# youmi-zym/TemporalStereo

Hardware: AMD Instinct MI355X
Metric: stereo pairs/sec, FlyingThings3D 540x960 D=192 (aggregation hot path) (higher is better)
Workload: dtype f32

## Files before the change

### include/ts_hip.h

```cpp
#ifndef TS_HIP_H
#define TS_HIP_H

#include <stddef.h>
#include <stdint.h>

#ifdef __cplusplus
extern "C" {
#endif

#define TS_OK 0
#define TS_ERR_NULL (-1)
#define TS_ERR_SHAPE (-2)
#define TS_ERR_UNSUPPORTED (-3)
#define TS_ERR_ALIGN (-4)

int ts_version(void);
const char* ts_last_error_string(void);

size_t ts_block_cost_workspace_bytes(int B, int C, int H, int W, int D, int scales);

int ts_block_cost_int_fwd(const float* left, const float* right, float* out, void* workspace,
                          int B, int C, int H, int W, int D, int scales, void* stream);

int ts_block_cost_sampled_fwd(const float* left, const float* right, const float* disp, float* out,
// ... 377 lines not shown
                          long long dx_bstride, long long dx_cstride, void* stream);
int ts_conv3d_hw_bwd_weight(const float* x, const float* dy, float* dw, int B, int Cin, int Cout, int D, int H, int W,
                            int stride, int dilation, long long x_bstride, long long x_cstride, long long dy_bstride,
                            long long dy_cstride, void* workspace, size_t workspace_bytes, void* stream);
int ts_conv3d_d_bwd_data(const float* dy, const float* w_b, float* dx, int B, int Cin, int Cout, int Din, int H, int W,
                         int k, int stride, int dilation, int padding, int transposed, long long dy_bstride,
                         long long dy_cstride, long long dx_bstride, long long dx_cstride, void* stream);
int ts_conv3d_d_bwd_weight(const float* x, const float* dy, float* dw, int B, int Cin, int Cout, int Din, int H, int W,
                           int k, int stride, int dilation, int padding, long long x_bstride, long long x_cstride,
                           long long dy_bstride, long long dy_cstride, void* workspace, size_t workspace_bytes,
                           void* stream);
int ts_resize3d_add_act_fwd(const float* a, const float* add, float* out, int B, int C, int Da, int Ha, int Wa,
                            int D, int H, int W, int act, long long a_bstride, long long a_cstride,
                            long long add_bstride, long long add_cstride, long long out_bstride,
                            long long out_cstride, void* stream);
int ts_pool3d5_avgmax_fwd(const float* x, float* out_avg, float* out_max, int B, int C, int D, int H, int W,
                          long long x_bstride, long long x_cstride, long long avg_bstride, long long avg_cstride,
                          long long max_bstride, long long max_cstride, void* stream);
int ts_merge_candidates_fwd(const float* volume, const float* sample, const float* mem_sample, const float* mem_cost,
                            const float* past_w, const float* past_scale, const float* past_shift,
                            float* out_sample, float* out_volume, int B, int C, int D0, int K, int H, int W,
                            long long vol_bstride, long long vol_cstride, long long out_bstride,
                            long long out_cstride, void* stream);
int ts_convex_upsample_fwd(const float* mask, const float* disp, float* out, int B, int H, int W, int factor,
                           float disp_scale, void* stream);
int ts_convex_upsample_candidates_fwd(const float* mask, const float* disp, float* out, float* low, float* high,
                                      float* candidates, int B, int H, int W, int factor, float disp_scale, float range,
                                      int channel_offset, int channels_total, void* stream);
int ts_unet_upsample_fwd(const float* mask, const float* disp, float* out, int B, int h, int w, int Ho, int Wo,
                         void* stream);
int ts_convex_upsample_bwd(const float* mask, const float* disp, const float* grad_out, float* grad_mask, float* grad_disp,
                           int B, int H, int W, int factor, float disp_scale, void* stream);
int ts_unet_upsample_bwd(const float* mask, const float* disp, const float* grad_out, float* grad_mask, float* grad_disp,
                         void* workspace, int B, int h, int w, int Ho, int Wo, void* stream);
int ts_deconv2d_k4s2_fwd(const float* x, const float* w_t, const float* scale, const float* shift, float* y,
                         int B, int Cin, int Cout, int H, int W, int act, long long out_bstride, void* stream);
int ts_resize_bilinear_fwd(const float* x, float* out, int B, int C, int h, int w, int Ho, int Wo, float value_scale,
                           long long out_bstride, void* stream);
int ts_resize_bilinear_pair_fwd(const float* x0, const float* x1, float* out0, float* out1, int B, int C, int h, int w,
                                int Ho, int Wo, float value_scale0, float value_scale1, void* stream);
int ts_range_candidates_fwd(const float* disp, float* low, float* high, float* candidates, int B, int H, int W,
                            float range, int channel_offset, int channels_total, void* stream);

int ts_resize3d_add_act_bwd(const float* a, const float* add, const float* grad_out, float* grad_a, float* grad_add,
                            int B, int C, int Da, int Ha, int Wa, int D, int H, int W, int act, void* stream);
int ts_pool3d5_avgmax_bwd(const float* x, const float* grad_avg, const float* grad_max, float* grad_x,
// ... 43 lines not shown
```

### temporalstereo_amd/_lib.py

```python
import ctypes
import os
import threading

_HERE = os.path.dirname(os.path.abspath(__file__))
LIB_PATH = os.path.join(_HERE, "libts_hip.so")

_lock = threading.Lock()
_lib = None

c_f32p = ctypes.c_void_p
c_ptr = ctypes.c_void_p
c_int = ctypes.c_int
c_size = ctypes.c_size_t
c_float = ctypes.c_float

SIGNATURES = {
    "ts_version": (c_int, []),
    "ts_last_error_string": (ctypes.c_char_p, []),
    "ts_block_cost_workspace_bytes": (c_size, [c_int] * 6),
    "ts_block_cost_int_fwd": (c_int, [c_f32p, c_f32p, c_f32p, c_ptr] + [c_int] * 6 + [c_ptr]),
    "ts_block_cost_sampled_fwd": (c_int, [c_f32p, c_f32p, c_f32p, c_f32p, c_ptr] + [c_int] * 6 + [c_ptr]),
    "ts_block_cost_sampled_warped_fwd": (c_int, [c_f32p, c_f32p, c_f32p, c_f32p, c_ptr] + [c_int] * 6 + [c_ptr]),
    "ts_block_cost_sampled_corr_fwd": (c_int, [c_f32p, c_f32p, c_f32p, c_f32p, c_ptr] + [c_int] * 6 + [c_ptr]),
    "ts_block_cost_corr_split_supported": (c_int, [c_int] * 2),
# ... 103 lines not shown
    "ts_conv3d_hw_x6_weight_bytes": (ctypes.c_size_t, [c_int] * 2),
    "ts_conv3d_hw_x6_weight_split": (c_int, [c_f32p, c_ptr, c_int, c_int, c_ptr]),
    "ts_conv3d_hw_x6_weight_split_from": (c_int, [c_f32p, c_ptr, c_int, c_int] + [ctypes.c_longlong] * 3 + [c_int, c_ptr]),
    "ts_conv3d_hw_x6_workspace_bytes": (c_size, [c_int] * 6),
    "ts_conv3d_hw_x6s_supported": (c_int, [c_int] * 5),
    "ts_conv3d_hw_x6s_weight_bytes": (c_size, [c_int] * 3),
    "ts_conv3d_hw_x6s_weight_split": (c_int, [c_f32p, c_ptr, c_int, c_int, c_int, c_int, c_ptr]),
    "ts_conv3d_hw_x6s_fwd": (c_int, [c_f32p, c_ptr, c_f32p, c_f32p, c_f32p] + [c_int] * 8 + [c_float] + [ctypes.c_longlong] * 4 + [c_ptr]),
    "ts_deconv2d_k4s2_unet_upsample_fwd": (c_int, [c_f32p, c_ptr, c_f32p, c_f32p, c_f32p, c_f32p] + [c_int] * 5 + [ctypes.c_longlong] * 2 + [c_ptr]),
    "ts_conv3d_hw_x6_fwd": (c_int, [c_f32p, c_ptr, c_f32p, c_f32p, c_f32p] + [c_int] * 8 + [c_float] + [ctypes.c_longlong] * 4 +
                            [c_f32p, ctypes.c_longlong, c_ptr, c_size, c_ptr]),
    "ts_conv3d_hw_fwd": (c_int, [c_f32p] * 5 + [c_int] * 10 + [c_float] + [ctypes.c_longlong] * 4 +
                         [c_f32p, ctypes.c_longlong, c_ptr, c_size, c_ptr]),
    "ts_conv3d_hw_workspace_bytes": (c_size, [c_int] * 8),
    "ts_conv3d_hw_bwd_data": (c_int, [c_f32p] * 3 + [c_int] * 9 + [ctypes.c_longlong] * 4 + [c_ptr]),
    "ts_conv3d_bwd_weight_workspace_bytes": (ctypes.c_size_t, [c_int] * 3),
    "ts_conv3d_hw_bwd_weight": (c_int, [c_f32p] * 3 + [c_int] * 8 + [ctypes.c_longlong] * 4 + [c_ptr, ctypes.c_size_t, c_ptr]),
    "ts_conv3d_d_bwd_data": (c_int, [c_f32p] * 3 + [c_int] * 11 + [ctypes.c_longlong] * 4 + [c_ptr]),
    "ts_conv3d_d_bwd_weight": (c_int, [c_f32p] * 3 + [c_int] * 10 + [ctypes.c_longlong] * 4 + [c_ptr, ctypes.c_size_t, c_ptr]),
    "ts_conv3d_d_fwd": (c_int, [c_f32p] * 5 + [c_int] * 12 + [c_float] + [ctypes.c_longlong] * 4 + [c_ptr]),
    "ts_resize3d_add_act_fwd": (c_int, [c_f32p] * 3 + [c_int] * 9 + [ctypes.c_longlong] * 6 + [c_ptr]),
    "ts_pool3d5_avgmax_fwd": (c_int, [c_f32p] * 3 + [c_int] * 5 + [ctypes.c_longlong] * 6 + [c_ptr]),
    "ts_merge_candidates_fwd": (c_int, [c_f32p] * 9 + [c_int] * 6 + [ctypes.c_longlong] * 4 + [c_ptr]),
    "ts_convex_upsample_fwd": (c_int, [c_f32p] * 3 + [c_int] * 4 + [c_float, c_ptr]),
    "ts_convex_upsample_candidates_fwd": (c_int, [c_f32p] * 6 + [c_int] * 4 + [c_float, c_float, c_int, c_int, c_ptr]),
    "ts_unet_upsample_fwd": (c_int, [c_f32p] * 3 + [c_int] * 5 + [c_ptr]),
    "ts_convex_upsample_bwd": (c_int, [c_f32p] * 5 + [c_int] * 4 + [c_float, c_ptr]),
    "ts_unet_upsample_bwd": (c_int, [c_f32p] * 5 + [c_ptr] + [c_int] * 5 + [c_ptr]),
    "ts_deconv2d_k4s2_fwd": (c_int, [c_f32p] * 5 + [c_int] * 6 + [ctypes.c_longlong, c_ptr]),
    "ts_resize_bilinear_fwd": (c_int, [c_f32p] * 2 + [c_int] * 6 + [c_float, ctypes.c_longlong, c_ptr]),
    "ts_resize_bilinear_pair_fwd": (c_int, [c_f32p] * 4 + [c_int] * 6 + [c_float, c_float, c_ptr]),
    "ts_range_candidates_fwd": (c_int, [c_f32p] * 4 + [c_int] * 3 + [c_float, c_int, c_int, c_ptr]),
    "ts_project_to_3d_fwd": (c_int, [c_f32p] * 7 + [c_int] * 6 + [c_float, c_ptr]),
    "ts_inverse_warp_fwd": (c_int, [c_f32p] * 9 + [c_ptr, c_f32p] + [c_int] * 11 + [c_float, c_ptr]),
    "ts_inverse_warp_bwd": (c_int, [c_f32p] * 8 + [c_int] * 11 + [c_float, c_ptr]),
    "ts_raft_corr_pyramid_fwd": (c_int, [c_f32p] * 3 + [c_int] * 5 + [c_ptr]),
    "ts_raft_corr_lookup_fwd": (c_int, [c_f32p] * 3 + [c_int] * 5 + [c_ptr]),
    "ts_raft_corr_lookup_bwd": (c_int, [c_f32p] * 5 + [c_int] * 6 + [c_ptr]),
    "ts_raft_corr_pyramid_bwd": (c_int, [c_f32p] * 5 + [c_int] * 5 + [c_ptr]),
    "ts_flow_corr_pyramid_fwd": (c_int, [c_f32p] * 3 + [c_int] * 5 + [c_ptr]),
    "ts_flow_corr_lookup_fwd": (c_int, [c_f32p] * 3 + [c_int] * 5 + [c_ptr]),
    "ts_flow_corr_lookup_bwd": (c_int, [c_f32p] * 5 + [c_int] * 6 + [c_ptr]),
    "ts_flow_corr_pyramid_bwd": (c_int, [c_f32p] * 5 + [c_int] * 5 + [c_ptr]),
    "ts_spp3d_pool_fwd": (c_int, [c_f32p] * 2 + [c_int] * 10 + [ctypes.c_longlong] * 2 + [c_ptr]),
    "ts_spp3d_pool_bwd": (c_int, [c_f32p] * 6 +[c_int] * 10 + [ctypes.c_longlong] * 4 + [c_ptr]),
    "ts_spp3d_expand_fwd": (c_int, [c_f32p] * 6 + [c_int] * 11 + [ctypes.c_longlong] * 2 + [c_ptr]),
# ... 7 lines not shown
    "ts_conv_gru_gate_bwd_a": (c_int, [c_f32p] * 7 + [c_int] * 2 + [ctypes.c_longlong] * 5 + [c_ptr]),
    "ts_conv_gru_gate_bwd_b": (c_int, [c_f32p] * 5 + [c_int] * 2 + [ctypes.c_longlong] * 7 + [c_ptr]),
    "ts_conv_gru_grad_sum": (c_int, [c_f32p] * 4 + [c_int] * 3 + [ctypes.c_longlong, c_ptr]),
    "ts_reproject_memory_workspace_bytes": (c_size, [c_int] * 5),
    "ts_reproject_memory_fwd": (c_int, [c_f32p, ctypes.c_longlong, c_int, c_int, c_f32p, c_f32p, c_int, c_f32p, c_int, c_int,
                                        c_f32p, c_int, c_f32p, c_f32p, c_f32p, c_float, c_float, c_f32p, c_f32p, c_f32p,
                                        c_ptr, c_int, c_int, c_int, c_ptr]),
    "ts_resize3d_add_act_bwd": (c_int, [c_f32p] * 5 + [c_int] * 9 + [c_ptr]),
    "ts_pool3d5_avgmax_bwd": (c_int, [c_f32p] * 4 + [c_int] * 5 + [c_ptr]),
    "ts_merge_candidates_bwd": (c_int, [c_f32p] * 5 + [c_int] * 5 + [c_ptr]),
    "ts_copy_rows_fwd": (c_int, [c_f32p] * 2 + [ctypes.c_longlong] * 4 + [c_ptr]),
    "ts_plan_create": (c_ptr, []),
    "ts_plan_destroy": (None, [c_ptr]),
    "ts_plan_length": (c_int, [c_ptr]),
    "ts_plan_add_call": (c_int, [c_ptr, ctypes.c_char_p, ctypes.POINTER(ctypes.c_ulonglong), c_int]),
    "ts_plan_run": (c_int, [c_ptr]),
    "ts_stream_fork": (c_int, [c_ptr, c_ptr]),
    "ts_event_record": (c_int, [c_int, c_ptr]),
    "ts_event_wait": (c_int, [c_int, c_ptr]),
}

_QUERIES = frozenset(n for n in SIGNATURES if n.endswith("_bytes") or n.startswith("ts_plan_") or
                     n.endswith("_split_supported") or
                     n in ("ts_version", "ts_last_error_string", "ts_conv_cout_pad", "ts_conv3d_hw_x6_supported", "ts_conv3d_hw_x6s_supported", "ts_peer_max_floats", "ts_peer_max_ranks",
                           "ts_peer_alloc", "ts_peer_open", "ts_peer_close", "ts_peer_free", "ts_peer_status", "ts_peer_status_async",
                           "ts_peer_set_timeout_ms", "ts_peer_reset", "ts_bn_set_small_elems",
                           "ts_conv_wgrad_defer", "ts_conv_wgrad_pending", "ts_conv_wgrad_take"))


def lib():
    rec = getattr(_tls, "recorder", None)
    if rec is not None:
        return rec.proxy
    return _real_lib()


def _real_lib():
    global _lib
    if _lib is None:
        with _lock:
            if _lib is None:
                if not os.path.exists(LIB_PATH):
                    raise RuntimeError(
                        "temporalstereo_amd: %s is missing -- build it with "
                        "`python -m temporalstereo_amd.build` (there is no fallback path)" % LIB_PATH)
                handle = ctypes.CDLL(LIB_PATH)
                for name, (res, args) in SIGNATURES.items():
# ... 115 lines not shown
```

### temporalstereo_amd/aggregation/native.py

```python
import os
import time

import torch
import torch.nn as nn

from .. import _lib
from .. import functional as TF

ACT_NONE, ACT_SILU, ACT_RELU, ACT_TANH_OFFSET, ACT_HEAD_PAIR = 0, 1, 2, 3, 4


def _stream():
    return _lib.current_stream_handle()


_PAR = {"on": False, "aux": None, "kinds": frozenset(__import__("os").environ.get("TS_BRANCHES", "hourglass").split(","))}


def _aux_stream():
    return _PAR["aux"]


_STAGE_CAP = int(os.environ.get("TS_STAGE_CHUNK_CAP", "8"))

# ... 421 lines not shown
    if split is not None:
        rc = _lib.lib().ts_conv3d_d_split_fwd(_lib.ptr(x), _lib.ptr(split), _lib.ptr(f.w), _lib.ptr(f.scale), _lib.ptr(f.shift),
                                              _lib.ptr(out), B, Cin, Cs, f.cout, Din, H, W, k, stride, dilation, padding,
                                              int(transposed), f.act if act is None else act, float(act_param),
                                              ib, ic, i2b, i2c, ob, oc, _stream())
        _lib.check(rc, "ts_conv3d_d_split_fwd")
        return out
    rc = _lib.lib().ts_conv3d_d_fwd(_lib.ptr(x), _lib.ptr(f.w), _lib.ptr(f.scale), _lib.ptr(f.shift), _lib.ptr(out),
                                    B, Cin, f.cout, Din, H, W, k, stride, dilation, padding, int(transposed),
                                    f.act if act is None else act, float(act_param), ib, ic, ob, oc, _stream())
    _lib.check(rc, "ts_conv3d_d_fwd")
    return out


FUSED_K1 = os.environ.get("TS_FUSED_K1", "1") != "0"
SPLIT_INPUT = os.environ.get("TS_SPLIT_INPUT", "1") != "0"
def _fused_tails(value):
    if value == "0":
        return frozenset()
    return frozenset(("convex", "deconv")) if value in ("", "1") else frozenset(value.split(","))


FUSED_TAILS = _fused_tails(os.environ.get("TS_FUSED_TAILS", "1"))


def block_cost_corr(left, right, disp, scales):
    return TF.block_cost_corr(left, right, disp, scales)


def conv_hw_warp(corr, f, q, disp, base, dilation=1):
    B, Cc, D, H, W = corr.shape
    assert Cc == f.cin, (Cc, f.cin)
    out = torch.empty((B, f.cout, D, H, W), device=corr.device, dtype=torch.float32)
    ib, ic = _strides5(corr)
    ob, oc = _strides5(out)
    wsb = TF._q("ts_conv3d_hw_warp_workspace_bytes", B, f.cout, D, H, W)
    ws = torch.empty(wsb, device=corr.device, dtype=torch.uint8)
    rc = _lib.lib().ts_conv3d_hw_warp_fwd(_lib.ptr(corr), _lib.ptr(f.w), _lib.ptr(f.scale), _lib.ptr(f.shift), _lib.ptr(out),
                                          _lib.ptr(q), _lib.ptr(disp), _lib.ptr(base), B, Cc, f.cout, D, H, W, dilation, f.act, 0.0,
                                          ib, ic, ob, oc, base.stride(0) if base is not None else 0, _lib.ptr(ws), wsb, _stream())
    _lib.check(rc, "ts_conv3d_hw_warp_fwd")
    return out


def resize_add_act(a, add, size, act=ACT_SILU):
    B, C, Da, Ha, Wa = a.shape
# ... 233 lines not shown
        y = conv_hw_warp(corr, self.init0_corr, rterm, ds, lterm.squeeze(2) if lterm.dim() == 5 else lterm, i0.dil)
        return conv_d(y, i0.f1, i0.k, i0.stride, i0.dil, i0.pad_d, i0.transposed)

    def init3d_from(self, first):
        return self.init2(self.hg(first))

    def feature_terms(self, left, right):
        return self.left_term(left), (self.right_term(right) if FUSED_K1 else None)


class _MergingLevel(_LevelBase):
    def __init__(self, mod):
        super().__init__(mod)
        pc = mod.past_conv
        f = fold_wrapper(pc, "d")
        self.past_w = f.w.reshape(-1)[:self.C].contiguous()
        self.past_scale, self.past_shift = f.scale[:self.C].contiguous(), f.shift[:self.C].contiguous()
        self.fusion = mod.spatial_fusion
        if self.fusion:
            self.conv5 = fold_wrapper(mod.fuse.conv_5x5, "d")
            self.fuse_conv = SepConv(mod.fuse.conv_fuse)
        self.up = ConvexUp(mod.convex_upsample)

    def merge(self, vol, samples, prev_info, resize_memory):
        B, C, D0, H, W = vol.shape
        K = self.topk
        memory = prev_info.get('cost_memory', None)
        mem_s = mem_c = None
        if memory is not None and prev_info.get('use_past_cost', False):
            mem_s, mem_c = memory['disp_sample'], memory['cost_volume']
            if resize_memory:
                mem_s, mem_c = resize_bilinear_pair(mem_s, mem_c, (H, W), W / mem_s.shape[-1], 1.0)
            mem_s, mem_c = _lib.contiguous(mem_s), _lib.contiguous(mem_c)
        Dm = D0 + K
        nch = 4 * C if self.fusion else C
        cat4 = torch.empty((B, nch, Dm, H, W), device=vol.device, dtype=torch.float32)
        samp = torch.empty((B, Dm, H, W), device=vol.device, dtype=torch.float32)
        x0 = cat4[:, :C]
        vb, vc = _strides5(vol); ob, oc = _strides5(x0)
        rc = _lib.lib().ts_merge_candidates_fwd(_lib.ptr(vol), _lib.ptr(samples), _lib.ptr(mem_s), _lib.ptr(mem_c),
                                                _lib.ptr(self.past_w), _lib.ptr(self.past_scale), _lib.ptr(self.past_shift),
                                                _lib.ptr(samp), _lib.ptr(x0), B, C, D0, K, H, W, vb, vc, ob, oc, _stream())
        _lib.check(rc, "ts_merge_candidates_fwd")
        return cat4, samp

    def fuse(self, cat4):
        C = self.C
        x0 = cat4[:, :C]
        if not self.fusion:
            return x0
        br = Branch("pool")
        with br:
            pool5(x0, cat4[:, 2 * C:3 * C], cat4[:, 3 * C:])
        conv_d(x0, self.conv5, 5, 1, 1, 2, out=cat4[:, C:2 * C])
        br.join()
        return self.fuse_conv(cat4)

    def merge_fuse_predict(self, vol, samples, prev_info, feat, resize_memory, mask=None, next_range=None):
        cat4, samp = self.merge(vol, samples, prev_info, resize_memory)
        cost, off = self.heads(self.fuse(cat4))
        if "convex" in FUSED_TAILS and next_range is not None and self.up.r <= 8:
            if callable(mask):
                mask = mask()
            return self.up.regress_with_candidates(feat, cost, samp, off, self.topk, mask, *next_range), cost, off, samp
        disp, _, _ = TF.topk_softargmax(cost, samp, off, k=self.topk)
        if callable(mask):
            mask = mask()
        if next_range is not None:
            return self.up.with_candidates(feat, disp, mask, *next_range), cost, off, samp
        return self.up(feat, disp, mask), cost, off, samp


class NativeCoarse(_MergingLevel):
# ... 407 lines not shown
```

### temporalstereo_amd/csrc/plan.hip

```cpp
#include <cstdint>
#include <cstring>
#include <mutex>
#include <string>
#include <utility>
#include <vector>

#include "ts_common.hpp"

namespace {

constexpr int kMaxWords = 32;

template <class T>
T unpack(unsigned long long w) {
  static_assert(sizeof(T) <= sizeof(unsigned long long), "argument wider than a plan word");
  T v;
  std::memcpy(&v, &w, sizeof(T));
  return v;
}

template <class... A, size_t... I>
int call_with(int (*f)(A...), const unsigned long long* w, std::index_sequence<I...>) {
  return f(unpack<A>(w[I])...);
}
// ... 56 lines not shown
    TS_PLAN_OP(ts_space_to_depth2_fwd),
    TS_PLAN_OP(ts_deconv2d_k4s2_weight_to_conv3), TS_PLAN_OP(ts_deconv2d_k4s2_wgrad_from_conv3),
    TS_PLAN_OP(ts_clip_rmsprop_step),       TS_PLAN_OP(ts_bn_sync_merge),
    TS_PLAN_OP(ts_bn_fold_many),
    TS_PLAN_OP(ts_conv_weight_layout_many2), TS_PLAN_OP(ts_conv_wgrad_finish_many), TS_PLAN_OP(ts_channel_sum_fwd),
    TS_PLAN_OP(ts_block_cost_sampled_warped_bwd),
    TS_PLAN_OP(ts_frames_prepare_fwd),      TS_PLAN_OP(ts_intrinsics_pyramid_fwd),  TS_PLAN_OP(ts_disp_u16_decode_fwd),
    TS_PLAN_OP(ts_frames_augment_fwd),      TS_PLAN_OP(ts_disp_u16_window_fwd),
    TS_PLAN_OP(ts_block_cost_sampled_corr_split_fwd), TS_PLAN_OP(ts_conv3d_hw_split_fwd),
    TS_PLAN_OP(ts_conv3d_d_split_fwd),      TS_PLAN_OP(ts_conv3d_hw_x6_split_fwd),
    TS_PLAN_OP(ts_inverse_warp_fwd),        TS_PLAN_OP(ts_inverse_warp_bwd),
    TS_PLAN_OP(ts_raft_corr_pyramid_fwd),   TS_PLAN_OP(ts_raft_corr_lookup_fwd),
    TS_PLAN_OP(ts_raft_corr_lookup_bwd),    TS_PLAN_OP(ts_raft_corr_pyramid_bwd),
    TS_PLAN_OP(ts_flow_corr_pyramid_fwd),   TS_PLAN_OP(ts_flow_corr_lookup_fwd),
    TS_PLAN_OP(ts_flow_corr_lookup_bwd),    TS_PLAN_OP(ts_flow_corr_pyramid_bwd),
    TS_PLAN_OP(ts_flow_metrics_fwd),        TS_PLAN_OP(ts_flow_render_fwd),         TS_PLAN_OP(ts_flow_u16_decode_fwd),
    TS_PLAN_OP(ts_spp3d_pool_fwd),          TS_PLAN_OP(ts_spp3d_pool_bwd),
    TS_PLAN_OP(ts_spp3d_expand_fwd),        TS_PLAN_OP(ts_spp3d_expand_bwd),        TS_PLAN_OP(ts_depth_sum3_fwd),
    TS_PLAN_OP(ts_bn_small_train_bwd),
    TS_PLAN_OP(ts_regress_convex_upsample_fwd), TS_PLAN_OP(ts_topk_softargmax_half_fwd),
    TS_PLAN_OP(ts_deconv2d_k4s2_unet_upsample_fwd),
    TS_PLAN_OP(ts_conv_gru_weight_layout),  TS_PLAN_OP(ts_conv_gru_gates_fwd),      TS_PLAN_OP(ts_conv_gru_out_fwd),
    TS_PLAN_OP(ts_conv_gru_gate_bwd_a),     TS_PLAN_OP(ts_conv_gru_gate_bwd_b),     TS_PLAN_OP(ts_conv_gru_grad_sum),
};

struct Call {
  const Entry* op;
  unsigned long long w[kMaxWords];
};

__global__ void __launch_bounds__(256)
copy_rows_kernel(const float* __restrict__ src, float* __restrict__ dst, long long rows, long long row_elems,
                 long long src_pitch, long long dst_pitch) {
  const long long n = rows * row_elems;
  for (long long i = static_cast<long long>(blockIdx.x) * blockDim.x + threadIdx.x; i < n;
       i += static_cast<long long>(gridDim.x) * blockDim.x) {
    const long long r = i / row_elems, c = i - r * row_elems;
    dst[r * dst_pitch + c] = src[r * src_pitch + c];
  }
}

__global__ void __launch_bounds__(256)
copy_rows4_kernel(const float4* __restrict__ src, float4* __restrict__ dst, long long row_quads, long long src_pitch_q,
                  long long dst_pitch_q) {
  const float4* s = src + blockIdx.y * src_pitch_q;
  float4* d = dst + blockIdx.y * dst_pitch_q;
// ... 141 lines not shown
```

### temporalstereo_amd/csrc/pyramid_ops.hip

```cpp
#include "regress_tails.hpp"
#include "ts_common.hpp"

namespace {

__device__ __forceinline__ float silu(float v) {
#ifdef TS_EXACT_SILU
  return v / (1.f + expf(-v));
#endif
  const float d = 1.f + __builtin_amdgcn_exp2f(v * -1.4426950408889634f);
  const float r = __builtin_amdgcn_rcpf(d);
  const float rn = fmaf(fmaf(-d, r, 1.f), r, r);
  return v * (d < 3.0e38f ? rn : r);
}

unsigned grid_for(long long n, int threads) {
  long long blocks = (n + threads - 1) / threads;
  const long long cap = static_cast<long long>(ts::kNumCU) * 16;
  if (blocks > cap) blocks = cap;
  if (blocks < 1) blocks = 1;
  return static_cast<unsigned>(blocks);
}

unsigned exact_grid(long long n) { return static_cast<unsigned>((n + 255) / 256); }

// ... 25 lines not shown
    float ld, ly, lx;
    lin_src(p.sd, d, p.Da, d0, d1, ld);
    lin_src(p.sh, y, p.Ha, y0, y1, ly);
    lin_src(p.sw, x, p.Wa, x0, x1, lx);
    const size_t HWa = static_cast<size_t>(p.Ha) * p.Wa;
    const float* p0 = ap + d0 * HWa;
    const float* p1 = ap + d1 * HWa;
    const float v00 = (1.f - lx) * p0[y0 * p.Wa + x0] + lx * p0[y0 * p.Wa + x1];
    const float v01 = (1.f - lx) * p0[y1 * p.Wa + x0] + lx * p0[y1 * p.Wa + x1];
    const float v10 = (1.f - lx) * p1[y0 * p.Wa + x0] + lx * p1[y0 * p.Wa + x1];
    const float v11 = (1.f - lx) * p1[y1 * p.Wa + x0] + lx * p1[y1 * p.Wa + x1];
    float v = (1.f - ld) * ((1.f - ly) * v00 + ly * v01) + ld * ((1.f - ly) * v10 + ly * v11);
    if (bp) v += bp[i];
    op[i] = p.act == 1 ? silu(v) : v;
  }
}

constexpr int PT_Y = 8, PT_X = 32;
struct Pool5 {
  int C, D, H, W;
  long long x_bstride, x_cstride, avg_bstride, avg_cstride, max_bstride, max_cstride;
};

__global__ void __launch_bounds__(256)
pool5_avgmax_kernel(const float* __restrict__ x, float* __restrict__ oavg, float* __restrict__ omax, const Pool5 p) {
  __shared__ float tile_s[PT_Y + 4][PT_X + 4 + 1];
  __shared__ float tile_m[PT_Y + 4][PT_X + 4 + 1];
  const int tiles_x = (p.W + PT_X - 1) / PT_X;
  const int ty0 = (blockIdx.x / tiles_x) * PT_Y, tx0 = (blockIdx.x % tiles_x) * PT_X;
  const int c = blockIdx.y, b = blockIdx.z;
  const int tx = threadIdx.x & (PT_X - 1), ty = threadIdx.x / PT_X;
  const int y = ty0 + ty, xx = tx0 + tx;
  const size_t HW = static_cast<size_t>(p.H) * p.W;
  const float* xp = x + static_cast<size_t>(b) * p.x_bstride + static_cast<size_t>(c) * p.x_cstride;
  float* ap = oavg + static_cast<size_t>(b) * p.avg_bstride + static_cast<size_t>(c) * p.avg_cstride;
  float* mp = omax + static_cast<size_t>(b) * p.max_bstride + static_cast<size_t>(c) * p.max_cstride;
  constexpr int TW = PT_X + 4, TN = (PT_Y + 4) * TW;
  int soff[2], lidx[2];
  bool pad[2];
#pragma unroll
  for (int e = 0; e < 2; ++e) {
    const int i = min(static_cast<int>(threadIdx.x) + 256 * e, TN - 1);
    const int cx = i % TW, cy = i / TW;
    const int gy = ty0 + cy - 2, gx = tx0 + cx - 2;
    pad[e] = !(gy >= 0 && gy < p.H && gx >= 0 && gx < p.W);
    soff[e] = min(max(gy, 0), p.H - 1) * p.W + min(max(gx, 0), p.W - 1);
    lidx[e] = cy * (TW + 1) + cx;
  }
  float* tls = &tile_s[0][0];
  float* tlm = &tile_m[0][0];
  float nxt[2];
#pragma unroll
  for (int e = 0; e < 2; ++e) nxt[e] = xp[soff[e]];
  float rs[5], rm[5];
#pragma unroll
  for (int i = 0; i < 5; ++i) { rs[i] = 0.f; rm[i] = -INFINITY; }
  for (int d = 0; d < p.D + 2; ++d) {
    float s2 = 0.f, m2 = -INFINITY;
    if (d < p.D) {
      __syncthreads();
#pragma unroll
      for (int e = 0; e < 2; ++e) {
        tls[lidx[e]] = pad[e] ? 0.f : nxt[e];
        tlm[lidx[e]] = pad[e] ? -INFINITY : nxt[e];
      }
      __syncthreads();
      const int dn = min(d + 1, p.D - 1);
#pragma unroll
      for (int e = 0; e < 2; ++e) nxt[e] = xp[dn * HW + soff[e]];
#pragma unroll
      for (int ky = 0; ky < 5; ++ky)
#pragma unroll
        for (int kx = 0; kx < 5; ++kx) {
          s2 += tile_s[ty + ky][tx + kx];
          m2 = fmaxf(m2, tile_m[ty + ky][tx + kx]);
        }
    }
#pragma unroll
    for (int i = 0; i < 4; ++i) { rs[i] = rs[i + 1]; rm[i] = rm[i + 1]; }
    rs[4] = s2; rm[4] = m2;
    const int od = d - 2;
    if (od >= 0 && y < p.H && xx < p.W) {
      const float s = rs[0] + rs[1] + rs[2] + rs[3] + rs[4];
      const float m = fmaxf(fmaxf(fmaxf(rm[0], rm[1]), fmaxf(rm[2], rm[3])), rm[4]);
      const size_t o = od * HW + static_cast<size_t>(y) * p.W + xx;
      if (oavg) ap[o] = s * (1.f / 125.f);
      if (omax) mp[o] = m;
    }
  }
}

constexpr int MERGE_DMAX = 20;
struct Merge {
  int B, C, D0, K, HW;
  int implicit_samples;
  long long vol_bstride, vol_cstride, out_bstride, out_cstride;
};

constexpr int MERGE_CPB = 2;
// ... 30 lines not shown
      s[j] = p.implicit_samples ? static_cast<float>(j) : samp[(static_cast<size_t>(b) * p.D0 + jv) * p.HW + px];
      const float a = ms[mo];
      m[j] = mc[mo];
      if (j >= p.D0) s[j] = (j < DT) ? (has_mem ? a : 0.f) : INFINITY;
      if (!has_mem) m[j] = 0.f;
#pragma unroll
      for (int cc = 0; cc < MERGE_CPB; ++cc)
        v[j][cc] = vb[static_cast<size_t>(jv) * p.HW + static_cast<size_t>(min(c0 + cc, p.C - 1)) * p.vol_cstride];
    }
#pragma unroll
    for (int j = 0; j < DM; ++j) {
      int rank = 0;
#pragma unroll
      for (int q = 0; q < DM; ++q) rank += (s[q] < s[j]) || (s[q] == s[j] && q < j);
      if (j < DT) {
        if (c0 == 0) out_samp[(static_cast<size_t>(b) * DT + rank) * p.HW + px] = s[j];
        float* ov = out_vol + static_cast<size_t>(b) * p.out_bstride + static_cast<size_t>(rank) * p.HW + px;
#pragma unroll
        for (int cc = 0; cc < MERGE_CPB; ++cc) {
          const float val = (j < p.D0) ? v[j][cc] : silu(w_[cc] * m[j] * sc_[cc] + sh_[cc]);
          if (c0 + cc < p.C) ov[static_cast<size_t>(c0 + cc) * p.out_cstride] = val;
        }
      }
    }
  }
}

__global__ void __launch_bounds__(256)
convex_upsample_kernel(const float* __restrict__ mask, const float* __restrict__ disp, float* __restrict__ out,
                       int B, int H, int W, int r, float disp_scale,
                       float* __restrict__ low, float* __restrict__ high, float* __restrict__ cand, float range, int coff, int ctot) {
  const int HW = H * W, Ho = H * r, Wo = W * r;
  const long long n = static_cast<long long>(B) * Ho * Wo;
  for (long long i = static_cast<long long>(blockIdx.x) * blockDim.x + threadIdx.x; i < n;
       i += static_cast<long long>(gridDim.x) * blockDim.x) {
    const int ox = static_cast<int>(i % Wo);
    const long long t = i / Wo;
    const int oy = static_cast<int>(t % Ho), b = static_cast<int>(t / Ho);
    const int y = oy / r, ry = oy - y * r, x = ox / r, rx = ox - x * r;
    const float* mp = mask + (static_cast<size_t>(b) * 9 * r * r + ry * r + rx) * HW + static_cast<size_t>(y) * W + x;
    const float* dp = disp + static_cast<size_t>(b) * HW;
    float m[9];
    const float mx = ts_tail::convex_logits(mp, static_cast<size_t>(r) * r * HW, m);
    const float dup = ts_tail::convex_combine(m, mx, [&](int k) {
      const int yy = y + k / 3 - 1, xx = x + k % 3 - 1;
      const float dv = dp[min(max(yy, 0), H - 1) * W + min(max(xx, 0), W - 1)];
// ... 364 lines not shown
}

extern "C" int ts_merge_candidates_fwd(const float* volume, const float* sample, const float* mem_sample, const float* mem_cost,
                                       const float* past_w, const float* past_scale, const float* past_shift,
                                       float* out_sample, float* out_volume, int B, int C, int D0, int K, int H, int W,
                                       long long vol_bstride, long long vol_cstride, long long out_bstride,
                                       long long out_cstride, void* stream) {
  TS_REQUIRE(B > 0 && C > 0 && D0 > 0 && K >= 0 && H > 0 && W > 0, TS_ERR_SHAPE, "merge_candidates: non-positive size");
  TS_REQUIRE(D0 + K <= MERGE_DMAX, TS_ERR_UNSUPPORTED, "merge_candidates: more than %d candidates", MERGE_DMAX);
  TS_REQUIRE_PTR(volume); TS_REQUIRE_PTR(out_sample); TS_REQUIRE_PTR(out_volume);
  if (K > 0) { TS_REQUIRE_PTR(past_w); TS_REQUIRE_PTR(past_scale); TS_REQUIRE_PTR(past_shift); }
  Merge p;
  p.B = B; p.C = C; p.D0 = D0; p.K = K; p.HW = H * W; p.implicit_samples = sample ? 0 : 1;
  p.vol_bstride = vol_bstride; p.vol_cstride = vol_cstride; p.out_bstride = out_bstride; p.out_cstride = out_cstride;
  const dim3 grid(grid_for(static_cast<long long>(B) * H * W, 256), (C + MERGE_CPB - 1) / MERGE_CPB);
#define TS_MERGE(DMV)                                                                                              \
  hipLaunchKernelGGL(merge_candidates_kernel<DMV>, grid, dim3(256), 0, ts::as_stream(stream), volume, sample,      \
                     mem_sample, mem_cost, past_w, past_scale, past_shift, out_sample, out_volume, p)
  if (D0 + K <= 8) TS_MERGE(8);
  else if (D0 + K <= 14) TS_MERGE(14);
  else TS_MERGE(MERGE_DMAX);
#undef TS_MERGE
  return ts::launched("merge_candidates_kernel");
}

namespace {
__global__ void __launch_bounds__(256)
convex_upsample_bwd_mask_kernel(const float* __restrict__ mask, const float* __restrict__ disp, const float* __restrict__ g,
                                float* __restrict__ gmask, int B, int H, int W, int r, float disp_scale) {
  const int HW = H * W, Ho = H * r, Wo = W * r;
  const long long n = static_cast<long long>(B) * Ho * Wo;
  const long long i = static_cast<long long>(blockIdx.x) * blockDim.x + threadIdx.x;
  if (i >= n) return;
  const int ox = static_cast<int>(i % Wo);
  const long long t = i / Wo;
  const int oy = static_cast<int>(t % Ho), b = static_cast<int>(t / Ho);
  const int y = oy / r, ry = oy - y * r, x = ox / r, rx = ox - x * r;
  const size_t base = (static_cast<size_t>(b) * 9 * r * r + ry * r + rx) * HW + static_cast<size_t>(y) * W + x;
  const float* dp = disp + static_cast<size_t>(b) * HW;
  float m[9], v[9], mx = -INFINITY;
#pragma unroll
  for (int k = 0; k < 9; ++k) { m[k] = mask[base + static_cast<size_t>(k) * r * r * HW]; mx = fmaxf(mx, m[k]); }
  float den = 0.f, acc = 0.f;
#pragma unroll
  for (int k = 0; k < 9; ++k) {
    m[k] = expf(m[k] - mx);
// ... 276 lines not shown
```

### temporalstereo_amd/csrc/ts_common.hpp

```cpp
#pragma once
#include <hip/hip_runtime.h>

#include <cstdarg>
#include <cstdint>
#include <cstdio>
#include <cstdlib>
#include <type_traits>

#include "../../include/ts_hip.h"

#define TS_ABI_VERSION 20

namespace ts {

char* err_buf();
int fail(int code, const char* fmt, ...);

inline hipStream_t as_stream(void* s) { return reinterpret_cast<hipStream_t>(s); }

inline bool aligned16(const void* p) { return (reinterpret_cast<uintptr_t>(p) & 15u) == 0; }

inline size_t round_up(size_t v, size_t a) { return (v + a - 1) / a * a; }

inline int launched(const char* what) {
  hipError_t e = hipGetLastError();
  if (e != hipSuccess) return fail(static_cast<int>(e), "%s: %s", what, hipGetErrorString(e));
  return TS_OK;
}

template <class F>
inline void dispatch_bool(bool b, F&& f) {
  if (b) f(std::true_type{});
  else f(std::false_type{});
}
// ... 23 lines not shown
```

Measured before the change: 1625.

## Fuse candidate merge with 5x5x5 avg/max pooling and make pool5 separable

Adds an optional kernel that sorts and merges candidates and computes the avg/max pool of the merged volume in one pass. This avoids re-reading the merged volume in a separate pool kernel. The existing pool5 kernel now computes horizontal partial sums and maxes in shared memory before the vertical reduction, which cuts shared-memory reads but adds barriers. The fused path is off unless TS_MERGE_POOL is set.

Result: slower. 1567 (-3.6%).

```diff
diff --git a/include/ts_hip.h b/include/ts_hip.h
--- a/include/ts_hip.h
+++ b/include/ts_hip.h
@@ -423,6 +423,13 @@
                             float* out_sample, float* out_volume, int B, int C, int D0, int K, int H, int W,
                             long long vol_bstride, long long vol_cstride, long long out_bstride,
                             long long out_cstride, void* stream);
+int ts_merge_pool5_supported(int D0, int K);
+int ts_merge_pool5_fwd(const float* volume, const float* sample, const float* mem_sample, const float* mem_cost,
+                       const float* past_w, const float* past_scale, const float* past_shift, float* out_sample,
+                       float* out_volume, float* out_avg, float* out_max, int B, int C, int D0, int K, int H, int W,
+                       long long vol_bstride, long long vol_cstride, long long out_bstride, long long out_cstride,
+                       long long avg_bstride, long long avg_cstride, long long max_bstride, long long max_cstride,
+                       void* stream);
 int ts_convex_upsample_fwd(const float* mask, const float* disp, float* out, int B, int H, int W, int factor,
                            float disp_scale, void* stream);
 int ts_convex_upsample_candidates_fwd(const float* mask, const float* disp, float* out, float* low, float* high,
diff --git a/temporalstereo_amd/_lib.py b/temporalstereo_amd/_lib.py
--- a/temporalstereo_amd/_lib.py
+++ b/temporalstereo_amd/_lib.py
@@ -149,6 +149,8 @@
     "ts_resize3d_add_act_fwd": (c_int, [c_f32p] * 3 + [c_int] * 9 + [ctypes.c_longlong] * 6 + [c_ptr]),
     "ts_pool3d5_avgmax_fwd": (c_int, [c_f32p] * 3 + [c_int] * 5 + [ctypes.c_longlong] * 6 + [c_ptr]),
     "ts_merge_candidates_fwd": (c_int, [c_f32p] * 9 + [c_int] * 6 + [ctypes.c_longlong] * 4 + [c_ptr]),
+    "ts_merge_pool5_supported": (c_int, [c_int] * 2),
+    "ts_merge_pool5_fwd": (c_int, [c_f32p] * 11 + [c_int] * 6 + [ctypes.c_longlong] * 8 + [c_ptr]),
     "ts_convex_upsample_fwd": (c_int, [c_f32p] * 3 + [c_int] * 4 + [c_float, c_ptr]),
     "ts_convex_upsample_candidates_fwd": (c_int, [c_f32p] * 6 + [c_int] * 4 + [c_float, c_float, c_int, c_int, c_ptr]),
     "ts_unet_upsample_fwd": (c_int, [c_f32p] * 3 + [c_int] * 5 + [c_ptr]),
@@ -202,7 +204,7 @@
 
 _QUERIES = frozenset(n for n in SIGNATURES if n.endswith("_bytes") or n.startswith("ts_plan_") or
                      n.endswith("_split_supported") or
-                     n in ("ts_version", "ts_last_error_string", "ts_conv_cout_pad", "ts_conv3d_hw_x6_supported", "ts_conv3d_hw_x6s_supported", "ts_peer_max_floats", "ts_peer_max_ranks",
+                     n in ("ts_version", "ts_last_error_string", "ts_conv_cout_pad", "ts_conv3d_hw_x6_supported", "ts_conv3d_hw_x6s_supported", "ts_merge_pool5_supported", "ts_peer_max_floats", "ts_peer_max_ranks",
                            "ts_peer_alloc", "ts_peer_open", "ts_peer_close", "ts_peer_free", "ts_peer_status", "ts_peer_status_async",
                            "ts_peer_set_timeout_ms", "ts_peer_reset", "ts_bn_set_small_elems",
                            "ts_conv_wgrad_defer", "ts_conv_wgrad_pending", "ts_conv_wgrad_take"))
diff --git a/temporalstereo_amd/aggregation/native.py b/temporalstereo_amd/aggregation/native.py
--- a/temporalstereo_amd/aggregation/native.py
+++ b/temporalstereo_amd/aggregation/native.py
@@ -467,6 +467,7 @@
 
 
 FUSED_TAILS = _fused_tails(os.environ.get("TS_FUSED_TAILS", "1"))
+MERGE_POOL = os.environ.get("TS_MERGE_POOL", "0") not in ("0", "")
 
 
 def block_cost_corr(left, right, disp, scales):
@@ -746,6 +747,9 @@
             self.fuse_conv = SepConv(mod.fuse.conv_fuse)
         self.up = ConvexUp(mod.convex_upsample)
 
+    def pools_in_merge(self, Dm):
+        return bool(self.fusion and MERGE_POOL and _lib.lib().ts_merge_pool5_supported(Dm - self.topk, self.topk))
+
     def merge(self, vol, samples, prev_info, resize_memory):
         B, C, D0, H, W = vol.shape
         K = self.topk
@@ -762,6 +766,15 @@
         samp = torch.empty((B, Dm, H, W), device=vol.device, dtype=torch.float32)
         x0 = cat4[:, :C]
         vb, vc = _strides5(vol); ob, oc = _strides5(x0)
+        if self.pools_in_merge(Dm):
+            avg, mx = cat4[:, 2 * C:3 * C], cat4[:, 3 * C:]
+            ab, ac = _strides5(avg); mb, mc = _strides5(mx)
+            rc = _lib.lib().ts_merge_pool5_fwd(_lib.ptr(vol), _lib.ptr(samples), _lib.ptr(mem_s), _lib.ptr(mem_c),
+                                               _lib.ptr(self.past_w), _lib.ptr(self.past_scale), _lib.ptr(self.past_shift),
+                                               _lib.ptr(samp), _lib.ptr(x0), _lib.ptr(avg), _lib.ptr(mx), B, C, D0, K, H, W,
+                                               vb, vc, ob, oc, ab, ac, mb, mc, _stream())
+            _lib.check(rc, "ts_merge_pool5_fwd")
+            return cat4, samp
         rc = _lib.lib().ts_merge_candidates_fwd(_lib.ptr(vol), _lib.ptr(samples), _lib.ptr(mem_s), _lib.ptr(mem_c),
                                                 _lib.ptr(self.past_w), _lib.ptr(self.past_scale), _lib.ptr(self.past_shift),
                                                 _lib.ptr(samp), _lib.ptr(x0), B, C, D0, K, H, W, vb, vc, ob, oc, _stream())
@@ -773,6 +786,9 @@
         x0 = cat4[:, :C]
         if not self.fusion:
             return x0
+        if self.pools_in_merge(cat4.shape[2]):
+            conv_d(x0, self.conv5, 5, 1, 1, 2, out=cat4[:, C:2 * C])
+            return self.fuse_conv(cat4)
         br = Branch("pool")
         with br:
             pool5(x0, cat4[:, 2 * C:3 * C], cat4[:, 3 * C:])
diff --git a/temporalstereo_amd/csrc/plan.hip b/temporalstereo_amd/csrc/plan.hip
--- a/temporalstereo_amd/csrc/plan.hip
+++ b/temporalstereo_amd/csrc/plan.hip
@@ -102,6 +102,7 @@
     TS_PLAN_OP(ts_deconv2d_k4s2_unet_upsample_fwd),
     TS_PLAN_OP(ts_conv_gru_weight_layout),  TS_PLAN_OP(ts_conv_gru_gates_fwd),      TS_PLAN_OP(ts_conv_gru_out_fwd),
     TS_PLAN_OP(ts_conv_gru_gate_bwd_a),     TS_PLAN_OP(ts_conv_gru_gate_bwd_b),     TS_PLAN_OP(ts_conv_gru_grad_sum),
+    TS_PLAN_OP(ts_merge_pool5_fwd),
 };
 
 struct Call {
diff --git a/temporalstereo_amd/csrc/pyramid_ops.hip b/temporalstereo_amd/csrc/pyramid_ops.hip
--- a/temporalstereo_amd/csrc/pyramid_ops.hip
+++ b/temporalstereo_amd/csrc/pyramid_ops.hip
@@ -71,10 +71,58 @@
   long long x_bstride, x_cstride, avg_bstride, avg_cstride, max_bstride, max_cstride;
 };
 
+constexpr int PT_TW = PT_X + 4, PT_TN = (PT_Y + 4) * PT_TW, PT_LD = PT_TW + 1;
+
+__device__ __forceinline__ void pool5_tile_element(int e, int ty0, int tx0, int H, int W, int& soff, int& lidx, bool& pad) {
+  const int i = min(static_cast<int>(threadIdx.x) + 256 * e, PT_TN - 1);
+  const int cx = i % PT_TW, cy = i / PT_TW;
+  const int gy = ty0 + cy - 2, gx = tx0 + cx - 2;
+  pad = !(gy >= 0 && gy < H && gx >= 0 && gx < W);
+  soff = min(max(gy, 0), H - 1) * W + min(max(gx, 0), W - 1);
+  lidx = cy * PT_LD + cx;
+}
+
+__device__ __forceinline__ void pool5_plane_taps(float* __restrict__ tls, float* __restrict__ tlm, const int (&lidx)[2],
+                                                 const bool (&pad)[2], const float (&v)[2], int ty, int tx, float& s2, float& m2) {
+  __syncthreads();
+#pragma unroll
+  for (int e = 0; e < 2; ++e) {
+    tls[lidx[e]] = pad[e] ? 0.f : v[e];
+    tlm[lidx[e]] = pad[e] ? -INFINITY : v[e];
+  }
+  __syncthreads();
+  float hs[2] = {0.f, 0.f}, hm[2] = {-INFINITY, -INFINITY};
+#pragma unroll
+  for (int e = 0; e < 2; ++e)
+    if (e == 0 || ty < 4) {
+      const int o = (ty + PT_Y * e) * PT_LD + tx;
+#pragma unroll
+      for (int kx = 0; kx < 5; ++kx) {
+        hs[e] += tls[o + kx];
+        hm[e] = fmaxf(hm[e], tlm[o + kx]);
+      }
+    }
+  __syncthreads();
+#pragma unroll
+  for (int e = 0; e < 2; ++e)
+    if (e == 0 || ty < 4) {
+      const int o = (ty + PT_Y * e) * PT_LD + tx;
+      tls[o] = hs[e];
+      tlm[o] = hm[e];
+    }
+  __syncthreads();
+  s2 = 0.f; m2 = -INFINITY;
+#pragma unroll
+  for (int ky = 0; ky < 5; ++ky) {
+    s2 += tls[(ty + ky) * PT_LD + tx];
+    m2 = fmaxf(m2, tlm[(ty + ky) * PT_LD + tx]);
+  }
+}
+
 __global__ void __launch_bounds__(256)
 pool5_avgmax_kernel(const float* __restrict__ x, float* __restrict__ oavg, float* __restrict__ omax, const Pool5 p) {
-  __shared__ float tile_s[PT_Y + 4][PT_X + 4 + 1];
-  __shared__ float tile_m[PT_Y + 4][PT_X + 4 + 1];
+  __shared__ float tile_s[PT_Y + 4][PT_LD];
+  __shared__ float tile_m[PT_Y + 4][PT_LD];
   const int tiles_x = (p.W + PT_X - 1) / PT_X;
   const int ty0 = (blockIdx.x / tiles_x) * PT_Y, tx0 = (blockIdx.x % tiles_x) * PT_X;
   const int c = blockIdx.y, b = blockIdx.z;
@@ -84,18 +132,10 @@
   const float* xp = x + static_cast<size_t>(b) * p.x_bstride + static_cast<size_t>(c) * p.x_cstride;
   float* ap = oavg + static_cast<size_t>(b) * p.avg_bstride + static_cast<size_t>(c) * p.avg_cstride;
   float* mp = omax + static_cast<size_t>(b) * p.max_bstride + static_cast<size_t>(c) * p.max_cstride;
-  constexpr int TW = PT_X + 4, TN = (PT_Y + 4) * TW;
   int soff[2], lidx[2];
   bool pad[2];
 #pragma unroll
-  for (int e = 0; e < 2; ++e) {
-    const int i = min(static_cast<int>(threadIdx.x) + 256 * e, TN - 1);
-    const int cx = i % TW, cy = i / TW;
-    const int gy = ty0 + cy - 2, gx = tx0 + cx - 2;
-    pad[e] = !(gy >= 0 && gy < p.H && gx >= 0 && gx < p.W);
-    soff[e] = min(max(gy, 0), p.H - 1) * p.W + min(max(gx, 0), p.W - 1);
-    lidx[e] = cy * (TW + 1) + cx;
-  }
+  for (int e = 0; e < 2; ++e) pool5_tile_element(e, ty0, tx0, p.H, p.W, soff[e], lidx[e], pad[e]);
   float* tls = &tile_s[0][0];
   float* tlm = &tile_m[0][0];
   float nxt[2];
@@ -107,23 +147,11 @@
   for (int d = 0; d < p.D + 2; ++d) {
     float s2 = 0.f, m2 = -INFINITY;
     if (d < p.D) {
-      __syncthreads();
-#pragma unroll
-      for (int e = 0; e < 2; ++e) {
-        tls[lidx[e]] = pad[e] ? 0.f : nxt[e];
-        tlm[lidx[e]] = pad[e] ? -INFINITY : nxt[e];
-      }
-      __syncthreads();
+      const float cur[2] = {nxt[0], nxt[1]};
       const int dn = min(d + 1, p.D - 1);
 #pragma unroll
       for (int e = 0; e < 2; ++e) nxt[e] = xp[dn * HW + soff[e]];
-#pragma unroll
-      for (int ky = 0; ky < 5; ++ky)
-#pragma unroll
-        for (int kx = 0; kx < 5; ++kx) {
-          s2 += tile_s[ty + ky][tx + kx];
-          m2 = fmaxf(m2, tile_m[ty + ky][tx + kx]);
-        }
+      pool5_plane_taps(tls, tlm, lidx, pad, cur, ty, tx, s2, m2);
     }
 #pragma unroll
     for (int i = 0; i < 4; ++i) { rs[i] = rs[i + 1]; rm[i] = rm[i + 1]; }
@@ -200,6 +228,109 @@
           if (c0 + cc < p.C) ov[static_cast<size_t>(c0 + cc) * p.out_cstride] = val;
         }
       }
+    }
+  }
+}
+
+constexpr int MERGE_POOL_DMAX = 16;
+struct MergePool {
+  int C, D0, K, H, W;
+  int implicit_samples;
+  long long vol_bstride, vol_cstride, out_bstride, out_cstride, avg_bstride, avg_cstride, max_bstride, max_cstride;
+};
+
+template <int DM>
+__global__ void __launch_bounds__(256)
+merge_pool5_kernel(const float* __restrict__ vol, const float* __restrict__ samp, const float* __restrict__ mem_samp,
+                   const float* __restrict__ mem_cost, const float* __restrict__ pw, const float* __restrict__ pscale,
+                   const float* __restrict__ pshift, float* __restrict__ out_samp, float* __restrict__ out_vol,
+                   float* __restrict__ oavg, float* __restrict__ omax, const MergePool p) {
+  __shared__ float tile_s[PT_Y + 4][PT_LD];
+  __shared__ float tile_m[PT_Y + 4][PT_LD];
+  const int DT = p.D0 + p.K;
+  const int tiles_x = (p.W + PT_X - 1) / PT_X;
+  const int ty0 = (blockIdx.x / tiles_x) * PT_Y, tx0 = (blockIdx.x % tiles_x) * PT_X;
+  const int c = blockIdx.y, b = blockIdx.z;
+  const int tx = threadIdx.x & (PT_X - 1), ty = threadIdx.x / PT_X;
+  const int y = ty0 + ty, xx = tx0 + tx;
+  const size_t HW = static_cast<size_t>(p.H) * p.W;
+  const bool has_mem = mem_samp != nullptr && mem_cost != nullptr && p.K > 0;
+  const int Kc = max(p.K, 1);
+  const float* vp = vol + static_cast<size_t>(b) * p.vol_bstride + static_cast<size_t>(c) * p.vol_cstride;
+  const float* sp = p.implicit_samples ? vol : samp + static_cast<size_t>(b) * p.D0 * HW;
+  const float* msp = has_mem ? mem_samp + static_cast<size_t>(b) * p.K * HW : vol;
+  const float* mcp = has_mem ? mem_cost + static_cast<size_t>(b) * p.K * HW : vol;
+  float* xo = out_vol + static_cast<size_t>(b) * p.out_bstride + static_cast<size_t>(c) * p.out_cstride;
+  float* ap = oavg + static_cast<size_t>(b) * p.avg_bstride + static_cast<size_t>(c) * p.avg_cstride;
+  float* mp = omax + static_cast<size_t>(b) * p.max_bstride + static_cast<size_t>(c) * p.max_cstride;
+  const float w = p.K > 0 ? pw[c] : 0.f, sc = p.K > 0 ? pscale[c] : 0.f, sh = p.K > 0 ? pshift[c] : 0.f;
+  int soff[2], lidx[2];
+  bool pad[2], centre[2];
+  unsigned long long inv[2];
+#pragma unroll
+  for (int e = 0; e < 2; ++e) {
+    pool5_tile_element(e, ty0, tx0, p.H, p.W, soff[e], lidx[e], pad[e]);
+    const int i = static_cast<int>(threadIdx.x) + 256 * e;
+    const int cx = i % PT_TW, cy = i / PT_TW;
+    centre[e] = i < PT_TN && !pad[e] && cy >= 2 && cy < PT_Y + 2 && cx >= 2 && cx < PT_X + 2;
+    float s[DM];
+#pragma unroll
+    for (int j = 0; j < DM; ++j) {
+      const int jv = min(j, p.D0 - 1), jm = min(max(j - p.D0, 0), Kc - 1);
+      s[j] = p.implicit_samples ? static_cast<float>(j) : sp[static_cast<size_t>(jv) * HW + soff[e]];
+      const float a = msp[has_mem ? static_cast<size_t>(jm) * HW + soff[e] : 0];
+      if (j >= p.D0) s[j] = (j < DT) ? (has_mem ? a : 0.f) : INFINITY;
+    }
+    unsigned long long iv = 0;
+#pragma unroll
+    for (int j = 0; j < DM; ++j) {
+      int rank = 0;
+#pragma unroll
+      for (int q = 0; q < DM; ++q)
+        if (q != j) rank += (q < j) ? (s[q] <= s[j]) : (s[q] < s[j]);
+      if (j < DT) {
+        iv |= static_cast<unsigned long long>(j) << (4 * rank);
+        if (c == 0 && centre[e]) out_samp[(static_cast<size_t>(b) * DT + rank) * HW + soff[e]] = s[j];
+      }
+    }
+    inv[e] = iv;
+  }
+  float* tls = &tile_s[0][0];
+  float* tlm = &tile_m[0][0];
+  float col[DM][2];
+#pragma unroll
+  for (int d = 0; d < DM; ++d)
+#pragma unroll
+    for (int e = 0; e < 2; ++e) {
+      const int j = static_cast<int>((inv[e] >> (4 * d)) & 15);
+      const float v = vp[static_cast<size_t>(min(j, p.D0 - 1)) * HW + soff[e]];
+      const float mc = mcp[has_mem ? static_cast<size_t>(min(max(j - p.D0, 0), Kc - 1)) * HW + soff[e] : 0];
+      const float m = has_mem ? mc : 0.f;
+      col[d][e] = (j < p.D0) ? v : silu(w * m * sc + sh);
+    }
+  float rs[5], rm[5];
+#pragma unroll
+  for (int i = 0; i < 5; ++i) { rs[i] = 0.f; rm[i] = -INFINITY; }
+#pragma unroll
+  for (int d = 0; d < DM + 2; ++d) {
+    float s2 = 0.f, m2 = -INFINITY;
+    if (d < DM && d < DT) {
+      const float cur[2] = {col[d < DM ? d : 0][0], col[d < DM ? d : 0][1]};
+#pragma unroll
+      for (int e = 0; e < 2; ++e)
+        if (centre[e]) xo[d * HW + soff[e]] = cur[e];
+      pool5_plane_taps(tls, tlm, lidx, pad, cur, ty, tx, s2, m2);
+    }
+#pragma unroll
+    for (int i = 0; i < 4; ++i) { rs[i] = rs[i + 1]; rm[i] = rm[i + 1]; }
+    rs[4] = s2; rm[4] = m2;
+    const int od = d - 2;
+    if (od >= 0 && od < DT && y < p.H && xx < p.W) {
+      const float s = rs[0] + rs[1] + rs[2] + rs[3] + rs[4];
+      const float m = fmaxf(fmaxf(fmaxf(rm[0], rm[1]), fmaxf(rm[2], rm[3])), rm[4]);
+      const size_t o = od * HW + static_cast<size_t>(y) * p.W + xx;
+      ap[o] = s * (1.f / 125.f);
+      mp[o] = m;
     }
   }
 }
@@ -610,6 +741,35 @@
   else TS_MERGE(MERGE_DMAX);
 #undef TS_MERGE
   return ts::launched("merge_candidates_kernel");
+}
+
+extern "C" int ts_merge_pool5_supported(int D0, int K) { return D0 > 0 && K >= 0 && D0 + K <= MERGE_POOL_DMAX; }
+
+extern "C" int ts_merge_pool5_fwd(const float* volume, const float* sample, const float* mem_sample, const float* mem_cost,
+                                  const float* past_w, const float* past_scale, const float* past_shift, float* out_sample,
+                                  float* out_volume, float* out_avg, float* out_max, int B, int C, int D0, int K, int H, int W,
+                                  long long vol_bstride, long long vol_cstride, long long out_bstride, long long out_cstride,
+                                  long long avg_bstride, long long avg_cstride, long long max_bstride, long long max_cstride,
+                                  void* stream) {
+  TS_REQUIRE(B > 0 && C > 0 && D0 > 0 && K >= 0 && H > 0 && W > 0, TS_ERR_SHAPE, "merge_pool5: non-positive size");
+  TS_REQUIRE(ts_merge_pool5_supported(D0, K), TS_ERR_UNSUPPORTED, "merge_pool5: more than %d candidates", MERGE_POOL_DMAX);
+  TS_REQUIRE(B <= 65535 && C <= 65535, TS_ERR_UNSUPPORTED, "merge_pool5: grid too large");
+  TS_REQUIRE(static_cast<long long>(H) * W < (1ll << 31), TS_ERR_UNSUPPORTED, "merge_pool5: plane too large");
+  TS_REQUIRE_PTR(volume); TS_REQUIRE_PTR(out_sample); TS_REQUIRE_PTR(out_volume); TS_REQUIRE_PTR(out_avg); TS_REQUIRE_PTR(out_max);
+  if (K > 0) { TS_REQUIRE_PTR(past_w); TS_REQUIRE_PTR(past_scale); TS_REQUIRE_PTR(past_shift); }
+  MergePool p;
+  p.C = C; p.D0 = D0; p.K = K; p.H = H; p.W = W; p.implicit_samples = sample ? 0 : 1;
+  p.vol_bstride = vol_bstride; p.vol_cstride = vol_cstride; p.out_bstride = out_bstride; p.out_cstride = out_cstride;
+  p.avg_bstride = avg_bstride; p.avg_cstride = avg_cstride; p.max_bstride = max_bstride; p.max_cstride = max_cstride;
+  const dim3 grid(((H + PT_Y - 1) / PT_Y) * ((W + PT_X - 1) / PT_X), C, B);
+#define TS_MERGE_POOL(DMV)                                                                                         \
+  hipLaunchKernelGGL(merge_pool5_kernel<DMV>, grid, dim3(256), 0, ts::as_stream(stream), volume, sample,           \
+                     mem_sample, mem_cost, past_w, past_scale, past_shift, out_sample, out_volume, out_avg, out_max, p)
+  if (D0 + K <= 8) TS_MERGE_POOL(8);
+  else if (D0 + K <= 14) TS_MERGE_POOL(14);
+  else TS_MERGE_POOL(MERGE_POOL_DMAX);
+#undef TS_MERGE_POOL
+  return ts::launched("merge_pool5_kernel");
 }
 
 namespace {
diff --git a/temporalstereo_amd/csrc/ts_common.hpp b/temporalstereo_amd/csrc/ts_common.hpp
--- a/temporalstereo_amd/csrc/ts_common.hpp
+++ b/temporalstereo_amd/csrc/ts_common.hpp
@@ -9,7 +9,7 @@
 
 #include "../../include/ts_hip.h"
 
-#define TS_ABI_VERSION 20
+#define TS_ABI_VERSION 21
 
 namespace ts {
 
```
